# Prisma-pResearch/Deep_Interpolation_Clustering

Measured on AMD Instinct MI355X. Metric: encounters/sec per joint interp+DEC step, higher is better.
Workload: dtype bf16; 1 GPU; 75000 synthetic encounters/GPU, 6 vitals, ~50 irregular samples per channel per 24h (T=96), R=24, K=4, loss ae_mse+10*kl [BASELINE.json configs[1]]; every epoch walks the WHOLE cohort behind a fresh permutation: 3 batches of 32768 incl. the last of 9464 (no drop_last, as upstream); value = encounters stepped / s; ms_per_step = mean over those steps; per_gpu_batch=32768, global_batch=32768, batches_per_epoch=3, encounters_stepped=16242232, parallelism=single, index_order=shuffled, input=ragged encounter store read in place (208 MB resident)

## Files before the change

deep_interpolation_clustering_amd/csrc/dic_lstmgrad.hip:

```cpp
#include "dic_common.h"

namespace dic {

constexpr int GH = 128;
constexpr int G4 = 4 * GH;
constexpr int XW = 32;
constexpr int TR = 32;
constexpr int NBUF = 3;
#ifndef DIC_DW_DGPAD
#define DIC_DW_DGPAD 64
#endif
constexpr int DG_PITCH = 2 * G4 + DIC_DW_DGPAD;
constexpr int H_PITCH = 2 * GH;
constexpr int X_PITCH = 2 * XW;
constexpr int LDS_DG = TR * DG_PITCH, LDS_H = TR * H_PITCH, LDS_X = TR * X_PITCH;
constexpr int SLOT = LDS_DG + LDS_H + LDS_X;
constexpr int WT_COLS = 19, WT_PITCH = 2 * G4 + 16;
constexpr int LDS_WT = WT_COLS * WT_PITCH;
constexpr int LDS_RED = 2 * 4 * 1024;
constexpr int DW_LDS = NBUF * SLOT + LDS_WT + LDS_RED;

typedef __bf16 bf16x8 __attribute__((ext_vector_type(8)));
typedef short s16x4 __attribute__((ext_vector_type(4)));
typedef short s16x8 __attribute__((ext_vector_type(8)));
typedef float f32x16 __attribute__((ext_vector_type(16)));
typedef float f32x4 __attribute__((ext_vector_type(4)));

struct LstmParams {
    const float* w_ih[2]; const float* w_hh[2]; const float* b_ih[2]; const float* b_hh[2];
};
struct LstmGrads {
    float* w_ih[2]; float* w_hh[2]; float* b_ih[2]; float* b_hh[2];
};

template <typename T>
__global__ __launch_bounds__(256) void lstm_pack_kernel(LstmParams p, int I, int Ip, int bias_col, T* wih, T* whh, T* whh_t, T* bias, T* wih_t) {
    const int n_ih = 2 * G4 * Ip, n_hh = 2 * G4 * GH;
    const int total = n_ih + 2 * n_hh + 2 * G4 + (wih_t ? n_ih : 0);
    for (int i = blockIdx.x * 256 + threadIdx.x; i < total; i += gridDim.x * 256) {
        if (i >= n_ih + 2 * n_hh + 2 * G4) {
            const int j = i - (n_ih + 2 * n_hh + 2 * G4), c = j / (2 * G4), row = j - c * (2 * G4), d = row / G4, g = row - d * G4;
            float v = 0.f;
            if (c < I) v = p.w_ih[d][(size_t)g * I + c];
            else if (c == I && bias_col) v = p.b_ih[d][g] + p.b_hh[d][g];
            wih_t[j] = (T)v;
            continue;
        }
        if (i < n_ih) {
            const int row = i / Ip, c = i - row * Ip, d = row / G4, g = row - d * G4;
            float v = 0.f;
            if (c < I) v = p.w_ih[d][(size_t)g * I + c];
            else if (c == I && bias_col) v = p.b_ih[d][g] + p.b_hh[d][g];
            wih[i] = (T)v;
        } else if (i < n_ih + n_hh) {
            const int j = i - n_ih, d = j / (G4 * GH), k = j - d * (G4 * GH);
            whh[j] = (T)p.w_hh[d][k];
        } else if (i < n_ih + 2 * n_hh) {
            const int j = i - n_ih - n_hh, d = j / (G4 * GH), k = j - d * (G4 * GH), u = k / G4, n = k - u * G4;
            if (whh_t) whh_t[j] = (T)p.w_hh[d][(size_t)n * GH + u];
        } else {
            const int j = i - n_ih - 2 * n_hh, d = j / G4, g = j - d * G4;
            if (bias) bias[j] = (T)(p.b_ih[d][g] + p.b_hh[d][g]);
        }
    }
}

struct DwArgs {
    const __bf16* dg;
    const __bf16* hext;
    const __bf16* x;
    float* partials;
    const __bf16* wih;
    __bf16* dxp;
    int R, B;
};
typedef float f32x4_t __attribute__((ext_vector_type(4)));

__device__ __forceinline__ s16x4 lds_tr16(const unsigned char* p) {
    return __builtin_amdgcn_ds_read_tr16_b64_v4i16((__attribute__((address_space(3))) s16x4*)(p));
}
__device__ __forceinline__ void dma16(const void* sbase, unsigned voff, unsigned lds_dst) {
    unsigned keep;
    asm volatile("s_mov_b32 %0, m0\n\ts_mov_b32 m0, %3\n\ts_nop 0\n\tglobal_load_lds_dwordx4 %1, %2\n\ts_mov_b32 m0, %0"
                 : "=&s"(keep) : "v"(voff), "s"(sbase), "s"(lds_dst) : "memory");
}
__device__ __forceinline__ void dma4(const void* sbase, unsigned voff, unsigned lds_dst) {
    unsigned keep;
    asm volatile("s_mov_b32 %0, m0\n\ts_mov_b32 m0, %3\n\ts_nop 0\n\tglobal_load_lds_dword %1, %2\n\ts_mov_b32 m0, %0"
                 : "=&s"(keep) : "v"(voff), "s"(sbase), "s"(lds_dst) : "memory");
}

template <int XWT>
__global__ __launch_bounds__(512) void lstm_dw_kernel(DwArgs a) {
    static_assert(XWT == 32 || XWT == 64, "packed input rows are 32 or 64 wide");
    constexpr int NBX = XWT / 32, NBN = 4 + NBX;
    constexpr int NWT = GH + XWT;
    constexpr int XP = 2 * XWT, L_X = TR * XP;
    constexpr int SLOTT = LDS_DG + LDS_H + L_X;
    extern __shared__ __align__(16) unsigned char dwsm[];
    const int tid = threadIdx.x, lane = tid & 63;
    const int w = __builtin_amdgcn_readfirstlane(tid >> 6);
    const int dir = blockIdx.y;
    const long nrows = (long)a.R * a.B;
    const int ntiles = (int)((nrows + TR - 1) / TR), nch = gridDim.x;
    const __bf16* hsrc = a.hext + (dir ? (size_t)2 * a.B * 2 * GH + GH : 0);

    f32x16 acc[2][NBN];
#pragma unroll
    for (int mb = 0; mb < 2; ++mb)
#pragma unroll
        for (int nb = 0; nb < NBN; ++nb)
#pragma unroll
            for (int k = 0; k < 16; ++k) acc[mb][nb][k] = 0.f;

    const unsigned lds0 = (unsigned)(size_t)((__attribute__((address_space(3))) unsigned char*)dwsm);
    const unsigned v_dg = lane * 16;
    const unsigned v_h = (lane >> 4) * (2 * GH * 2) + (((lane & 15) ^ ((lane >> 4) << 2)) * 16);
    const unsigned v_x = lane * 4;
    const unsigned v_x64[2] = {(unsigned)((lane >> 5) * 128 + (((lane >> 4) & 1) * 64) + (lane & 15) * 4),
                               (unsigned)((lane >> 5) * 128 + ((((lane >> 4) & 1) ^ 1) * 64) + (lane & 15) * 4)};
    auto request = [&](int tile, int slot) {
        const long r0 = min((long)tile * TR, nrows - TR);
        const unsigned base = lds0 + slot * SLOTT;
#pragma unroll
        for (int p = 0; p < 4; ++p) {
            const int row = p * 8 + w;
            dma16(a.dg + ((size_t)(r0 + row) * 2 + dir) * G4, v_dg, base + row * DG_PITCH);
        }
        dma16(hsrc + (size_t)(r0 + w * 4) * 2 * GH, v_h, base + LDS_DG + w * 4 * H_PITCH);
        if constexpr (XWT == 32) {
            dma4(a.x + (size_t)r0 * XWT + w * 128, v_x, base + LDS_DG + LDS_H + w * 256);
        } else {
#pragma unroll
            for (int i = 0; i < 2; ++i)
                dma4(a.x + (size_t)(r0 + 4 * w + 2 * i) * XWT, v_x64[i], base + LDS_DG + LDS_H + (4 * w + 2 * i) * XP);
        }
    };

    const int kq = (lane & 15) >> 2, kp = lane & 3, cb = (lane >> 4) & 1, hh = lane >> 5;
    const int rowoff = 8 * hh + kq;
    const int pa_off = rowoff * DG_PITCH + (64 * w + 16 * cb + 4 * kp) * 2;
    int px_off[NBX];
#pragma unroll
    for (int nbx = 0; nbx < NBX; ++nbx)
        px_off[nbx] = LDS_DG + LDS_H + rowoff * XP + (XWT == 64 ? ((nbx ^ ((rowoff >> 1) & 1)) * 64) : 0) + (16 * cb + 4 * kp) * 2;
    int ph_off[4];
#pragma unroll
    for (int nb = 0; nb < 4; ++nb) ph_off[nb] = LDS_DG + rowoff * H_PITCH + (((4 * nb + 2 * cb + (kp >> 1)) ^ (kq << 2)) * 16) + (kp & 1) * 8;
    auto frag = [&](const unsigned char* p, int pitch) {
        const s16x4 lo = lds_tr16(p), hi = lds_tr16(p + 4 * pitch);
        s16x8 f;
#pragma unroll
        for (int j = 0; j < 4; ++j) { f[j] = lo[j]; f[4 + j] = hi[j]; }
        return __builtin_bit_cast(bf16x8, f);
    };

    unsigned char* wt = dwsm + NBUF * SLOTT;
    float* red = reinterpret_cast<float*>(wt + LDS_WT);
    const bool want_dx = XWT == 32 && a.wih != nullptr;
    if (want_dx) {
        for (int i = tid; i < WT_COLS * G4; i += 512) {
            const int xc = i / G4, k = i - xc * G4;
            *reinterpret_cast<__bf16*>(wt + xc * WT_PITCH + k * 2) = a.wih[((size_t)dir * G4 + k) * XWT + xc];
        }
    }
    const int q4 = w & 3, rw = q4 >> 1, xcb = q4 & 1, khalf = w >> 2, li = lane & 15, kq4 = lane >> 4;
    const int dxa_off = (16 * rw + li) * DG_PITCH + (khalf * 256 + 8 * kq4) * 2;
    const int dxb_off = min(16 * xcb + li, WT_COLS - 1) * WT_PITCH + (khalf * 256 + 8 * kq4) * 2;
    long prev_r0 = -1;
    int parity = 0;
    f32x4_t own_prev = {0.f, 0.f, 0.f, 0.f};
    auto finish_dx = [&](int par, long r0p) {
        if (want_dx && khalf == 0 && r0p >= 0) {
            const f32x4_t o = *reinterpret_cast<const f32x4_t*>(red + (par * 4 + q4) * 256 + lane * 4);
            __bf16* dst = a.dxp + ((size_t)dir * nrows + r0p + 16 * rw + 4 * kq4) * XWT + 16 * xcb + li;
#pragma unroll
            for (int e = 0; e < 4; ++e) dst[(size_t)e * XWT] = (__bf16)(o[e] + own_prev[e]);
        }
    };

    int tile = blockIdx.x, slot = 0;
    if (tile < ntiles) request(tile, 0);
    if (tile + nch < ntiles) request(tile + nch, 1);
    for (; tile < ntiles; tile += nch) {
        if (tile + nch < ntiles) {
            if constexpr (XWT == 32) asm volatile("s_waitcnt vmcnt(6) lgkmcnt(0)" ::: "memory");
            else asm volatile("s_waitcnt vmcnt(7) lgkmcnt(0)" ::: "memory");
        } else {
            asm volatile("s_waitcnt vmcnt(0) lgkmcnt(0)" ::: "memory");
        }
        __builtin_amdgcn_s_barrier();
        finish_dx(parity ^ 1, prev_r0);
        if (tile + 2 * nch < ntiles) request(tile + 2 * nch, slot == 0 ? 2 : slot - 1);
        unsigned char* base = dwsm + slot * SLOTT;
        if ((long)tile * TR + TR > nrows) {
            const int dup = (int)((long)tile * TR + TR - nrows);
            for (int i = tid; i < dup * (H_PITCH + XP) / 16; i += 512) {
                const int nh = dup * H_PITCH / 16;
                unsigned char* dst = i < nh ? base + LDS_DG + i * 16 : base + LDS_DG + LDS_H + (i - nh) * 16;
                *reinterpret_cast<uint4*>(dst) = make_uint4(0u, 0u, 0u, 0u);
            }
            asm volatile("s_waitcnt lgkmcnt(0)" ::: "memory");
            __builtin_amdgcn_s_barrier();
        }
#pragma unroll 1
        for (int ks = 0; ks < TR / 16; ++ks) {
            const unsigned char* kb = base + ks * 16 * DG_PITCH;
            bf16x8 af[2];
#pragma unroll
            for (int mb = 0; mb < 2; ++mb) af[mb] = frag(kb + pa_off + mb * 64, DG_PITCH);
#pragma unroll
            for (int nb = 0; nb < NBN; ++nb) {
                const bf16x8 bfg = nb < 4 ? frag(base + ks * 16 * H_PITCH + ph_off[nb < 4 ? nb : 0], H_PITCH)
                                          : frag(base + ks * 16 * XP + px_off[nb < 4 ? 0 : nb - 4], XP);
#pragma unroll
                for (int mb = 0; mb < 2; ++mb) acc[mb][nb] = __builtin_amdgcn_mfma_f32_32x32x16_bf16(af[mb], bfg, acc[mb][nb], 0, 0, 0);
            }
        }
        if (want_dx) {
            f32x4_t dacc = {0.f, 0.f, 0.f, 0.f};
#pragma unroll
            for (int ks = 0; ks < 8; ++ks) {
                const bf16x8 av = *reinterpret_cast<const bf16x8*>(base + dxa_off + ks * 64);
                const bf16x8 bv = *reinterpret_cast<const bf16x8*>(wt + dxb_off + ks * 64);
                dacc = __builtin_amdgcn_mfma_f32_16x16x32_bf16(av, bv, dacc, 0, 0, 0);
            }
            if (khalf) *reinterpret_cast<f32x4_t*>(red + (parity * 4 + q4) * 256 + lane * 4) = dacc;
            else own_prev = dacc;
            prev_r0 = min((long)tile * TR, nrows - TR);
            parity ^= 1;
        }
        slot = slot == NBUF - 1 ? 0 : slot + 1;
    }
    if (want_dx) {
        asm volatile("s_waitcnt lgkmcnt(0)" ::: "memory");
        __builtin_amdgcn_s_barrier();
        finish_dx(parity ^ 1, prev_r0);
    }
    float* o = a.partials + ((size_t)blockIdx.x * 2 + dir) * G4 * NWT;
#pragma unroll
    for (int mb = 0; mb < 2; ++mb)
#pragma unroll
        for (int nb = 0; nb < NBN; ++nb)
#pragma unroll
            for (int k = 0; k < 16; ++k) {
                const int m = 64 * w + 32 * mb + (k & 3) + 8 * (k >> 2) + 4 * hh;
                o[(size_t)m * NWT + 32 * nb + (lane & 31)] = acc[mb][nb][k];
            }
}

constexpr int DXW = 256;
constexpr int DNW = GH + DXW;
constexpr int DMH = G4 / 2;
static_assert(DNW / 32 == 12, "12 n-blocks = 2 wave groups x 6");
constexpr int WD_DG = TR * DMH * 2, WD_H = TR * GH * 2, WD_X = TR * DXW * 2;
constexpr int WD_SLOT = WD_DG + WD_H + WD_X;
constexpr int WD_LDS = NBUF * WD_SLOT;
constexpr int WD_OUT = 4 * DMH * DNW;

struct DwWideArgs {
    const __bf16* dg;
    const __bf16* hext;
    const __bf16* x;
    float* partials;
    int R, B;
    int x_relu;
};

__global__ __launch_bounds__(512) void lstm_dw_wide_kernel(DwWideArgs a) {
    extern __shared__ __align__(16) unsigned char dwsm[];
    const int tid = threadIdx.x, lane = tid & 63;
    const int w = __builtin_amdgcn_readfirstlane(tid >> 6);
    const int dir = blockIdx.y >> 1, mh = blockIdx.y & 1;
    const long nrows = (long)a.R * a.B;
    const int ntiles = (int)((nrows + TR - 1) / TR), nch = gridDim.x;
    const __bf16* hsrc = a.hext + (dir ? (size_t)2 * a.B * 2 * GH + GH : 0);
    const __bf16* gsrc = a.dg + (size_t)dir * G4 + mh * DMH;

    const int mg = w & 3, ng = w >> 2;
    f32x16 acc[2][6];
#pragma unroll
    for (int mb = 0; mb < 2; ++mb)
#pragma unroll
        for (int nb = 0; nb < 6; ++nb)
#pragma unroll
            for (int k = 0; k < 16; ++k) acc[mb][nb][k] = 0.f;

    const unsigned lds0 = (unsigned)(size_t)((__attribute__((address_space(3))) unsigned char*)dwsm);
    const int r2 = lane >> 5, sw2 = ((2 * (w & 1) + r2) & 3) << 2;
    const unsigned v_dg = r2 * (2 * G4 * 2) + (((lane & 31) ^ sw2) * 16);
    const unsigned v_x = r2 * (DXW * 2) + (((lane & 31) ^ sw2) * 16);
    const unsigned v_h = (lane >> 4) * (2 * GH * 2) + (((lane & 15) ^ ((lane >> 4) << 2)) * 16);
    auto request = [&](int tile, int slot) {
        const long r0 = min((long)tile * TR, nrows - TR);
        const unsigned base = lds0 + slot * WD_SLOT;
#pragma unroll
        for (int p = 0; p < 2; ++p) {
            const int row = 2 * (w + 8 * p);
            dma16(gsrc + (size_t)(r0 + row) * 2 * G4, v_dg, base + row * (DMH * 2));
            dma16(a.x + (size_t)(r0 + row) * DXW, v_x, base + WD_DG + WD_H + row * (DXW * 2));
        }
        dma16(hsrc + (size_t)(r0 + w * 4) * 2 * GH, v_h, base + WD_DG + w * 4 * (GH * 2));
    };

    const int kq = (lane & 15) >> 2, kp = lane & 3, cb = (lane >> 4) & 1, hh = lane >> 5;
    const int rowoff = 8 * hh + kq;
    auto piece = [&](int j) { return (((4 * j + 2 * cb + (kp >> 1)) ^ (kq << 2)) * 16) + (kp & 1) * 8; };
    int pa_off[2], pb_off[6], pb_pitch[6];
    short pb_floor[6];
#pragma unroll
    for (int mb = 0; mb < 2; ++mb) pa_off[mb] = rowoff * (DMH * 2) + piece(2 * mg + mb);
#pragma unroll
    for (int i = 0; i < 6; ++i) {
        const int j = 6 * ng + i;
        pb_pitch[i] = j < 4 ? GH * 2 : DXW * 2;
        pb_floor[i] = (j >= 4 && a.x_relu) ? (short)0 : (short)-32768;
        pb_off[i] = j < 4 ? WD_DG + rowoff * (GH * 2) + piece(j) : WD_DG + WD_H + rowoff * (DXW * 2) + piece(j - 4);
    }
    auto frag = [&](const unsigned char* p, int pitch) {
        const s16x4 lo = lds_tr16(p), hi = lds_tr16(p + 4 * pitch);
        s16x8 f;
#pragma unroll
        for (int j = 0; j < 4; ++j) { f[j] = lo[j]; f[4 + j] = hi[j]; }
        return __builtin_bit_cast(bf16x8, f);
    };

    int tile = blockIdx.x, slot = 0;
    if (tile < ntiles) request(tile, 0);
    if (tile + nch < ntiles) request(tile + nch, 1);
    for (; tile < ntiles; tile += nch) {
        if (tile + nch < ntiles) asm volatile("s_waitcnt vmcnt(5) lgkmcnt(0)" ::: "memory");
        else asm volatile("s_waitcnt vmcnt(0) lgkmcnt(0)" ::: "memory");
        __builtin_amdgcn_s_barrier();
        if (tile + 2 * nch < ntiles) request(tile + 2 * nch, slot == 0 ? 2 : slot - 1);
        unsigned char* base = dwsm + slot * WD_SLOT;
        if ((long)tile * TR + TR > nrows) {
            const int dup = (int)((long)tile * TR + TR - nrows);
            const int nh = dup * GH * 2 / 16, nx = dup * DXW * 2 / 16;
            for (int i = tid; i < nh + nx; i += 512) {
                unsigned char* dst = i < nh ? base + WD_DG + i * 16 : base + WD_DG + WD_H + (i - nh) * 16;
                *reinterpret_cast<uint4*>(dst) = make_uint4(0u, 0u, 0u, 0u);
            }
            asm volatile("s_waitcnt lgkmcnt(0)" ::: "memory");
            __builtin_amdgcn_s_barrier();
        }
#ifdef DIC_DWW_EXP_NOMMA
        const int nks = a.R < 0 ? 1 : 0;
#else
        const int nks = TR / 16;
#endif
#pragma unroll 1
        for (int ks = 0; ks < nks; ++ks) {
            bf16x8 af[2];
#pragma unroll
            for (int mb = 0; mb < 2; ++mb) af[mb] = frag(base + ks * 16 * (DMH * 2) + pa_off[mb], DMH * 2);
#pragma unroll
            for (int i = 0; i < 6; ++i) {
                bf16x8 bfg = frag(base + ks * 16 * pb_pitch[i] + pb_off[i], pb_pitch[i]);
                {
                    typedef short s16x8v __attribute__((ext_vector_type(8)));
                    const short fl = pb_floor[i];
                    const s16x8v flv = {fl, fl, fl, fl, fl, fl, fl, fl};
                    bfg = __builtin_bit_cast(bf16x8, __builtin_elementwise_max(__builtin_bit_cast(s16x8v, bfg), flv));
                }
#pragma unroll
                for (int mb = 0; mb < 2; ++mb) acc[mb][i] = __builtin_amdgcn_mfma_f32_32x32x16_bf16(af[mb], bfg, acc[mb][i], 0, 0, 0);
            }
        }
        slot = slot == NBUF - 1 ? 0 : slot + 1;
    }
    float* o = a.partials + ((size_t)blockIdx.x * 4 + blockIdx.y) * DMH * DNW;
#pragma unroll
    for (int mb = 0; mb < 2; ++mb)
#pragma unroll
        for (int i = 0; i < 6; ++i)
#pragma unroll
            for (int k = 0; k < 16; ++k) {
                const int m = 64 * mg + 32 * mb + (k & 3) + 8 * (k >> 2) + 4 * hh;
                o[(size_t)m * DNW + 32 * (6 * ng + i) + (lane & 31)] = acc[mb][i][k];
            }
}

__global__ __launch_bounds__(256) void lstm_dw_wide_finalize(const float* partials, int nch, LstmGrads g, float beta) {
    const int i = (blockIdx.x * 256 + threadIdx.x) * 4;
    if (i >= WD_OUT) return;
    double ch[8][4];
#pragma unroll
    for (int k = 0; k < 8; ++k)
#pragma unroll
        for (int e = 0; e < 4; ++e) ch[k][e] = 0.0;
    const float* src = partials + i;
    int b = 0;
    for (; b + 8 <= nch; b += 8) {
        float4 v[8];
#pragma unroll
        for (int k = 0; k < 8; ++k) v[k] = *reinterpret_cast<const float4*>(src + (size_t)(b + k) * WD_OUT);
#pragma unroll
        for (int k = 0; k < 8; ++k) { ch[k][0] += (double)v[k].x; ch[k][1] += (double)v[k].y; ch[k][2] += (double)v[k].z; ch[k][3] += (double)v[k].w; }
    }
    for (; b < nch; ++b) {
        const float4 v = *reinterpret_cast<const float4*>(src + (size_t)b * WD_OUT);
        ch[0][0] += (double)v.x; ch[0][1] += (double)v.y; ch[0][2] += (double)v.z; ch[0][3] += (double)v.w;
    }
    const int part = i / (DMH * DNW), rem = i - part * (DMH * DNW), m = (part & 1) * DMH + rem / DNW, n = rem % DNW, d = part >> 1;
    float* dst = n < GH ? g.w_hh[d] + (size_t)m * GH + n : g.w_ih[d] + (size_t)m * DXW + (n - GH);
#pragma unroll
    for (int e = 0; e < 4; ++e) {
        const double s = ((ch[0][e] + ch[1][e]) + (ch[2][e] + ch[3][e])) + ((ch[4][e] + ch[5][e]) + (ch[6][e] + ch[7][e]));
        dst[e] = beta != 0.f ? fmaf(beta, dst[e], (float)s) : (float)s;
    }
}
static_assert(WD_OUT % 4 == 0 && DNW % 4 == 0 && GH % 4 == 0, "four outputs per thread");

static int dw_wide_chunks(int R, int B) {
    const int ntiles = (int)(((long)R * B + TR - 1) / TR);
    const int n = max(1, min(ntiles, kNumCU / 4));
    return n >= 8 ? n / 8 * 8 : n;
}

__global__ __launch_bounds__(256) void lstm_dw_finalize(const float* partials, int nch, int I, int nw, LstmGrads g, float beta) {
    __shared__ double red[256];
    const int n_out = 2 * G4 * nw;
    const double s = reduce_partials_32x8(partials, nch, n_out, blockIdx.x * 32, red);
    const int i = blockIdx.x * 32 + threadIdx.x;
    if (threadIdx.x >= 32 || i >= n_out) return;
    const int d = i / (G4 * nw), rem = i - d * (G4 * nw), m = rem / nw, n = rem - m * nw;
    float* dst;
    if (n < GH) dst = g.w_hh[d] + (size_t)m * GH + n;
    else if (n - GH < I) dst = g.w_ih[d] + (size_t)m * I + (n - GH);
    else return;
    *dst = beta != 0.f ? fmaf(beta, *dst, (float)s) : (float)s;
}

__global__ __launch_bounds__(256) void lstm_unpack_grads_kernel(const float* dw_ih, int ldw, const float* dw_hh, const float* dbias,
                                                               int I, LstmGrads g, float beta) {
    const int n_ih = dw_ih ? 2 * G4 * I : 0, n_hh = dw_hh ? 2 * G4 * GH : 0, n_b = dbias ? 2 * G4 : 0;
    for (int i = blockIdx.x * 256 + threadIdx.x; i < n_ih + n_hh + n_b; i += gridDim.x * 256) {
        if (i < n_ih) {
            const int row = i / I, c = i - row * I, d = row / G4, m = row - d * G4;
            float* dst = g.w_ih[d] + (size_t)m * I + c;
            const float v = dw_ih[(size_t)row * ldw + c];
            *dst = beta != 0.f ? fmaf(beta, *dst, v) : v;
        } else if (i < n_ih + n_hh) {
            const int j = i - n_ih, d = j / (G4 * GH), k = j - d * (G4 * GH);
            float* dst = g.w_hh[d] + k;
            *dst = beta != 0.f ? fmaf(beta, *dst, dw_hh[j]) : dw_hh[j];
        } else {
            const int j = i - n_ih - n_hh, d = j / G4, m = j - d * G4;
            const float v = dbias[j];
            float* d1 = g.b_ih[d] + m;
            float* d2 = g.b_hh[d] + m;
            *d1 = beta != 0.f ? fmaf(beta, *d1, v) : v;
            *d2 = beta != 0.f ? fmaf(beta, *d2, v) : v;
        }
    }
}

constexpr int TX = 16;
template <int XWT, int DMH> struct DwX3 {
    static constexpr int NG = G4 / DMH;
    static constexpr int MW = DMH / 64;
    static constexpr int NBT = 4 + XWT / 32;
    static constexpr int NBN = (NBT + NG - 1) / NG;
    static constexpr int NWT = GH + XWT;
    static constexpr int DGP = DMH == G4 ? 2 * DMH + 64 : 2 * DMH;
    static constexpr int L_PL = TX * DGP, L_DG = 2 * L_PL;
    static constexpr int HP = 2 * GH + 64;
    static constexpr int XP = XWT == 32 ? 64 : 2 * XWT + 64;
    static constexpr int L_H = TX * HP, L_X = TX * XP;
    static constexpr int L_HX = 2 * L_H + 2 * L_X;
    static constexpr int L_RED = XWT == 32 ? 2 * 8 * 1024 : 0;
    static constexpr int LDS = 3 * L_DG + 2 * L_HX + L_RED;
    static constexpr int NXL = XWT == 32 ? 1 : 2;
    static constexpr int NDMA = DMH == G4 ? 4 : 2;
};

struct DwX3Args {
    const __bf16* dg;
    long dg_plane;
    const float* hext;
    const float* x;
    int ldx;
    float* partials;
    int R, B, x_relu;
    const float* wih;
    float* dxp;
};

__device__ __forceinline__ f32x4_t gload16(const void* sbase, unsigned voff) {
    f32x4_t v;
    asm volatile("global_load_dwordx4 %0, %1, %2" : "=&v"(v) : "v"(voff), "s"(sbase) : "memory");
    return v;
}
__device__ __forceinline__ void split4_store(unsigned char* hi, unsigned char* lo, f32x4_t v, bool relu, bool zero) {
    bf16x8 dummy; (void)dummy;
    typedef __bf16 b4 __attribute__((ext_vector_type(4)));
    b4 h, l;
#pragma unroll
    for (int j = 0; j < 4; ++j) {
        float x = zero ? 0.f : v[j];
        if (relu) x = fmaxf(x, 0.f);
        const __bf16 xh = (__bf16)x;
        h[j] = xh;
        l[j] = (__bf16)(x - (float)xh);
    }
    *reinterpret_cast<b4*>(hi) = h;
    *reinterpret_cast<b4*>(lo) = l;
}

#ifdef DIC_DWX3_EXP_TIMING
__device__ unsigned long long dic_dwx3_stamps[8][32][8];
#define DWX_STAMP(tile, slot)                                                                                         \
    do {                                                                                                              \
        if (blockIdx.x == 5 && blockIdx.y == 0 && (threadIdx.x & 63) == 0 && (tile) >= 8 && (tile) < 40)               \
            dic_dwx3_stamps[threadIdx.x >> 6][(tile) - 8][slot] = __builtin_readcyclecounter();                        \
    } while (0)
#else
#define DWX_STAMP(tile, slot) do {} while (0)
#endif

template <int XWT, int DMH>
__global__ __launch_bounds__(512) void lstm_dwx3_kernel(DwX3Args a) {
    typedef DwX3<XWT, DMH> C;
    extern __shared__ __align__(16) unsigned char dwsm[];
    const int tid = threadIdx.x, lane = tid & 63;
    const int w = __builtin_amdgcn_readfirstlane(tid >> 6);
    const int dir = blockIdx.y / C::NG, mh = blockIdx.y % C::NG;
    const int mg = w % C::MW, ng = w / C::MW;
    const long nrows = (long)a.R * a.B;
    const int ntiles = (int)((nrows + TX - 1) / TX), nch = gridDim.x;
    const int mine = (int)blockIdx.x < ntiles ? (ntiles - 1 - (int)blockIdx.x) / nch + 1 : 0;
    if (mine == 0) return;
    const float* hsrc = a.hext + (dir ? (size_t)2 * a.B * 2 * GH + GH : 0);
    const __bf16* gsrc = a.dg + (size_t)dir * G4 + mh * DMH;

    f32x16 acc[2][C::NBN];
#pragma unroll
    for (int mb = 0; mb < 2; ++mb)
#pragma unroll
        for (int nb = 0; nb < C::NBN; ++nb)
#pragma unroll
            for (int k = 0; k < 16; ++k) acc[mb][nb][k] = 0.f;

    unsigned char* const hx0 = dwsm + 3 * C::L_DG;
    const unsigned lds0 = (unsigned)(size_t)((__attribute__((address_space(3))) unsigned char*)dwsm);
    auto tile_r0 = [&](int j) { return min((long)((int)blockIdx.x + min(j, mine - 1) * nch) * TX, nrows - TX); };
    const int r2 = lane >> 5, sw2 = ((2 * (w & 1) + r2) & 3) << 2;
    const unsigned v_dg = DMH == G4 ? (unsigned)lane * 16 : (unsigned)(r2 * (2 * G4 * 2) + (((lane & 31) ^ sw2) * 16));
    auto request_dg = [&](int j) {
        const long r0 = tile_r0(j);
        const unsigned base = lds0 + (j % 3) * C::L_DG;
#pragma unroll
        for (int p = 0; p < 2; ++p) {
            const __bf16* src = gsrc + (size_t)p * a.dg_plane;
            if constexpr (DMH == G4) {
#pragma unroll
                for (int k = 0; k < 2; ++k) dma16(src + (size_t)(r0 + w + 8 * k) * 2 * G4, v_dg, base + p * C::L_PL + (w + 8 * k) * C::DGP);
            } else {
                dma16(src + (size_t)(r0 + 2 * w) * 2 * G4, v_dg, base + p * C::L_PL + 2 * w * C::DGP);
            }
        }
    };
    const int hrow = tid >> 5, hc4 = tid & 31;
    const unsigned v_h = (unsigned)(hrow * (2 * GH * 4) + hc4 * 16);
    const int xpc = a.ldx >> 2;
    int xrow[C::NXL], xc4[C::NXL];
    unsigned v_x[C::NXL];
    bool xon[C::NXL];
#pragma unroll
    for (int i = 0; i < C::NXL; ++i) {
        const int p = tid + 512 * i;
        xon[i] = p < TX * xpc;
        const int pc = xon[i] ? p : 0;
        xrow[i] = pc / xpc; xc4[i] = pc - xrow[i] * xpc;
        v_x[i] = (unsigned)((xrow[i] * a.ldx + 4 * xc4[i]) * 4);
    }
    const int h_pos = hrow * C::HP + hc4 * 8;
    int x_pos[C::NXL];
#pragma unroll
    for (int i = 0; i < C::NXL; ++i) x_pos[i] = xrow[i] * C::XP + xc4[i] * 8;
    f32x4_t hreg, xreg[C::NXL];
    auto request_hx = [&](int j) {
        const long r0 = tile_r0(j);
        hreg = gload16(hsrc + (size_t)r0 * 2 * GH, v_h);
#pragma unroll
        for (int i = 0; i < C::NXL; ++i) xreg[i] = gload16(a.x + (size_t)r0 * a.ldx, v_x[i]);
    };
    constexpr int NPIECE = 1 + C::NXL;
    static_assert(NPIECE <= C::NBN, "dwx3: one MFMA group per piece");
    auto store_piece = [&](int j, int pc) {
        const long t0 = (long)((int)blockIdx.x + min(j, mine - 1) * nch) * TX;
        const int dup = (int)max(0L, t0 + TX - nrows);
        unsigned char* base = hx0 + (j & 1) * C::L_HX;
        if (C::NBN >= 6 && dup == 0) {
            if (pc == 0) split4_store(base + h_pos, base + C::L_H + h_pos, hreg, false, false);
            else if (xon[pc - 1]) split4_store(base + 2 * C::L_H + x_pos[pc - 1], base + 2 * C::L_H + C::L_X + x_pos[pc - 1], xreg[pc - 1], a.x_relu != 0, false);
        } else if (pc == 0) {
            split4_store(base + h_pos, base + C::L_H + h_pos, hreg, false, h_pos < dup * C::HP);
        } else {
            const int i = pc - 1;
            if (xon[i]) split4_store(base + 2 * C::L_H + x_pos[i], base + 2 * C::L_H + C::L_X + x_pos[i], xreg[i], a.x_relu != 0, x_pos[i] < dup * C::XP);
        }
    };
    auto store_hx = [&](int j) {
#pragma unroll
        for (int pc = 0; pc < NPIECE; ++pc) store_piece(j, pc);
    };

    const int kq = (lane & 15) >> 2, kp = lane & 3, cb = (lane >> 4) & 1, hh = lane >> 5;
    const int rowoff = 8 * hh + kq;
    auto piece = [&](int j) { return (((4 * j + 2 * cb + (kp >> 1)) ^ (kq << 2)) * 16) + (kp & 1) * 8; };
    int pa_off[2], pb_pitch[C::NBN], pb_lo[C::NBN];
    int pb_sel[C::NBN], pb_soff[C::NBN];
    const int pb_h = rowoff * C::HP + (16 * cb + 4 * kp) * 2, pb_x = 2 * C::L_H + rowoff * C::XP + (16 * cb + 4 * kp) * 2;
#pragma unroll
    for (int mb = 0; mb < 2; ++mb)
        pa_off[mb] = DMH == G4 ? rowoff * C::DGP + (64 * mg + 32 * mb + 16 * cb + 4 * kp) * 2 : rowoff * C::DGP + piece(2 * mg + mb);
#pragma unroll
    for (int i = 0; i < C::NBN; ++i) {
        const int jn = min(C::NBN * ng + i, C::NBT - 1);
        pb_pitch[i] = jn < 4 ? C::HP : C::XP;
        pb_lo[i] = jn < 4 ? C::L_H : C::L_X;
        pb_sel[i] = jn < 4;
        pb_soff[i] = 64 * (jn < 4 ? jn : jn - 4);
    }
    auto pb_off = [&](int i) { return (pb_sel[i] ? pb_h : pb_x) + pb_soff[i]; };
    auto frag = [&](const unsigned char* p, int pitch) {
        const s16x4 lo = lds_tr16(p), hi = lds_tr16(p + 4 * pitch);
        s16x8 f;
#pragma unroll
        for (int j = 0; j < 4; ++j) { f[j] = lo[j]; f[4 + j] = hi[j]; }
        return __builtin_bit_cast(bf16x8, f);
    };

    constexpr bool DXOK = XWT == 32 && C::NG == 2;
    const bool want_dx = DXOK && a.wih != nullptr;
    float* red = reinterpret_cast<float*>(dwsm + 3 * C::L_DG + 2 * C::L_HX);
    bf16x8 wdh[2], wdl[2];
    const int li = lane & 15, kg4 = lane >> 4;
    if (want_dx) {
#pragma unroll
        for (int ks = 0; ks < 2; ++ks)
#pragma unroll
            for (int jj = 0; jj < 8; ++jj) {
                const int col = 16 * ng + li, k = mh * DMH + 64 * mg + 32 * ks + 8 * kg4 + jj;
                const float v = col < a.ldx ? a.wih[((size_t)dir * G4 + k) * a.ldx + col] : 0.f;
                const __bf16 vh = (__bf16)v;
                wdh[ks][jj] = vh;
                wdl[ks][jj] = (__bf16)(v - (float)vh);
            }
    }
    int dxa_off[2];
#pragma unroll
    for (int ks = 0; ks < 2; ++ks) dxa_off[ks] = li * C::DGP + (((8 * mg + 4 * ks + kg4) ^ ((li & 3) << 2)) * 16);
    auto finish_dx = [&](int jprev) {
        if (!want_dx || jprev < 0) return;
        const int row = tid >> 5, col = tid & 31;
        const float* src = red + (jprev & 1) * (8 * 256) + (col >> 4) * (4 * 256) + ((col & 15) + 16 * (row >> 2)) * 4 + (row & 3);
        const float sum = (src[0] + src[256]) + (src[512] + src[768]);
        if (col < a.ldx) a.dxp[((size_t)blockIdx.y * nrows + tile_r0(jprev) + row) * a.ldx + col] = sum;
    };

    if constexpr (XWT == 32) {
        for (int i = tid; i < 2 * C::L_HX / 16; i += 512) reinterpret_cast<uint4*>(hx0)[i] = make_uint4(0u, 0u, 0u, 0u);
        __syncthreads();
    }
    request_hx(0);
    request_dg(0);
    asm volatile("s_waitcnt vmcnt(%0)" :: "i"(C::NDMA) : "memory");
    asm volatile("" : "+v"(hreg));
#pragma unroll
    for (int i = 0; i < C::NXL; ++i) asm volatile("" : "+v"(xreg[i]));
    store_hx(0);
    request_hx(1);
    request_dg(1);
    for (int j = 0; j < mine; ++j) {
        DWX_STAMP(j, 0);
        asm volatile("s_waitcnt vmcnt(%0) lgkmcnt(0)" :: "i"(C::NDMA) : "memory");
        DWX_STAMP(j, 1);
        asm volatile("" : "+v"(hreg));
#pragma unroll
        for (int i = 0; i < C::NXL; ++i) asm volatile("" : "+v"(xreg[i]));
        __builtin_amdgcn_s_barrier();
        DWX_STAMP(j, 2);
        if constexpr (DXOK) finish_dx(j - 1);
        constexpr bool SPREAD = C::NBN >= 6;
        if constexpr (!SPREAD) {
            store_hx(j + 1);
            request_hx(j + 2);
            request_dg(j + 2);
        }
        DWX_STAMP(j, 3);
        DWX_STAMP(j, 4);
        const unsigned char* dgb = dwsm + (j % 3) * C::L_DG;
        const unsigned char* hxb = hx0 + (j & 1) * C::L_HX;
        bf16x8 ah[2], al[2];
#pragma unroll
        for (int mb = 0; mb < 2; ++mb) {
            ah[mb] = frag(dgb + pa_off[mb], C::DGP);
            al[mb] = frag(dgb + C::L_PL + pa_off[mb], C::DGP);
        }
        if constexpr (!SPREAD) {
#pragma unroll
            for (int i = 0; i < C::NBN; ++i) {
                const bf16x8 bh = frag(hxb + pb_off(i), pb_pitch[i]);
                const bf16x8 bl = frag(hxb + pb_off(i) + pb_lo[i], pb_pitch[i]);
#pragma unroll
                for (int mb = 0; mb < 2; ++mb) {
                    acc[mb][i] = __builtin_amdgcn_mfma_f32_32x32x16_bf16(ah[mb], bh, acc[mb][i], 0, 0, 0);
                    acc[mb][i] = __builtin_amdgcn_mfma_f32_32x32x16_bf16(al[mb], bh, acc[mb][i], 0, 0, 0);
                    acc[mb][i] = __builtin_amdgcn_mfma_f32_32x32x16_bf16(ah[mb], bl, acc[mb][i], 0, 0, 0);
                }
            }
        } else {
            bf16x8 bh = frag(hxb + pb_off(0), pb_pitch[0]);
            bf16x8 bl = frag(hxb + pb_off(0) + pb_lo[0], pb_pitch[0]);
    #pragma unroll
            for (int i = 0; i < C::NBN; ++i) {
                __builtin_amdgcn_sched_barrier(0);
    #pragma unroll
                for (int mb = 0; mb < 2; ++mb) acc[mb][i] = __builtin_amdgcn_mfma_f32_32x32x16_bf16(ah[mb], bh, acc[mb][i], 0, 0, 0);
    #pragma unroll
                for (int mb = 0; mb < 2; ++mb) acc[mb][i] = __builtin_amdgcn_mfma_f32_32x32x16_bf16(al[mb], bh, acc[mb][i], 0, 0, 0);
                __builtin_amdgcn_sched_barrier(0);
                if (i + 1 < C::NBN) bh = frag(hxb + pb_off(i + 1), pb_pitch[i + 1]);
                if constexpr (SPREAD) {
                    if (i < NPIECE) store_piece(j + 1, i);
                    if (i == NPIECE - 1) {
                        request_hx(j + 2);
                        request_dg(j + 2);
                    }
                }
                __builtin_amdgcn_sched_barrier(0);
    #pragma unroll
                for (int mb = 0; mb < 2; ++mb) acc[mb][i] = __builtin_amdgcn_mfma_f32_32x32x16_bf16(ah[mb], bl, acc[mb][i], 0, 0, 0);
                __builtin_amdgcn_sched_barrier(0);
                if (i + 1 < C::NBN) bl = frag(hxb + pb_off(i + 1) + pb_lo[i + 1], pb_pitch[i + 1]);
            }
            __builtin_amdgcn_sched_barrier(0);
        }
        DWX_STAMP(j, 5);
        if constexpr (DXOK) {
            if (want_dx) {
                f32x4_t d0 = {0.f, 0.f, 0.f, 0.f};
#pragma unroll
                for (int ks = 0; ks < 2; ++ks) {
                    const bf16x8 avh = *reinterpret_cast<const bf16x8*>(dgb + dxa_off[ks]);
                    const bf16x8 avl = *reinterpret_cast<const bf16x8*>(dgb + C::L_PL + dxa_off[ks]);
                    d0 = __builtin_amdgcn_mfma_f32_16x16x32_bf16(avh, wdh[ks], d0, 0, 0, 0);
                    d0 = __builtin_amdgcn_mfma_f32_16x16x32_bf16(avl, wdh[ks], d0, 0, 0, 0);
                    d0 = __builtin_amdgcn_mfma_f32_16x16x32_bf16(avh, wdl[ks], d0, 0, 0, 0);
                }
                *reinterpret_cast<f32x4_t*>(red + (j & 1) * (8 * 256) + (ng * 4 + mg) * 256 + lane * 4) = d0;
            }
        }
    }
    asm volatile("s_waitcnt vmcnt(0)" ::: "memory");
    if constexpr (DXOK) {
        if (want_dx) {
            asm volatile("s_waitcnt lgkmcnt(0)" ::: "memory");
            __builtin_amdgcn_s_barrier();
            finish_dx(mine - 1);
        }
    }
    float* o = a.partials + ((size_t)blockIdx.x * gridDim.y + blockIdx.y) * DMH * C::NWT;
#pragma unroll
    for (int mb = 0; mb < 2; ++mb)
#pragma unroll
        for (int i = 0; i < C::NBN; ++i) {
            if (C::NBN * ng + i >= C::NBT) continue;
#pragma unroll
            for (int k = 0; k < 16; ++k) {
                const int m = 64 * mg + 32 * mb + (k & 3) + 8 * (k >> 2) + 4 * hh;
                o[(size_t)m * C::NWT + 32 * (C::NBN * ng + i) + (lane & 31)] = acc[mb][i][k];
            }
        }
}

static int dw_chunks(int R, int B) {
    const int ntiles = (int)(((long)R * B + TR - 1) / TR);
    return max(1, min(ntiles, kNumCU / 2));
}
static int dwx3_chunks(int R, int B, bool wide) {
    const int ntiles = (int)(((long)R * B + TX - 1) / TX);
    (void)wide;
    const int n = max(1, min(ntiles, kNumCU / 4));
    return n >= 8 ? n / 8 * 8 : n;
}

}

using namespace dic;

extern "C" {

int dic_lstm_pack(int dtype, const float* const* params, int H, int I, int Ip, int bias_col, void* wih, void* whh, void* whh_t, void* bias,
                  void* wih_t, dic_stream_t stream) {
    DIC_REQUIRE(dtype == DIC_DTYPE_F32 || dtype == DIC_DTYPE_BF16, DIC_ERR_INVALID_ARG, "lstm_pack: dtype %d", dtype);
    DIC_REQUIRE(H == GH, DIC_ERR_UNSUPPORTED, "lstm_pack: hidden size %d (compiled for %d)", H, GH);
    DIC_REQUIRE(params && wih && whh, DIC_ERR_INVALID_ARG, "lstm_pack: NULL pointer");
    DIC_REQUIRE(I > 0 && Ip >= I + (bias_col ? 1 : 0) && Ip <= 1024, DIC_ERR_INVALID_ARG, "lstm_pack: I=%d Ip=%d bias_col=%d", I, Ip, bias_col);
    LstmParams p;
    for (int d = 0; d < 2; ++d) {
        p.w_ih[d] = params[4 * d + 0]; p.w_hh[d] = params[4 * d + 1]; p.b_ih[d] = params[4 * d + 2]; p.b_hh[d] = params[4 * d + 3];
        DIC_REQUIRE(p.w_ih[d] && p.w_hh[d] && p.b_ih[d] && p.b_hh[d], DIC_ERR_INVALID_ARG, "lstm_pack: NULL parameter (direction %d)", d);
    }
    const int total = 2 * G4 * Ip + 4 * G4 * GH + 2 * G4 + (wih_t ? 2 * G4 * Ip : 0);
    const dim3 grid(min((total + 255) / 256, 2 * kNumCU));
    if (dtype == DIC_DTYPE_BF16)
        hipLaunchKernelGGL(lstm_pack_kernel<__bf16>, grid, dim3(256), 0, (hipStream_t)stream, p, I, Ip, bias_col, (__bf16*)wih, (__bf16*)whh,
                           (__bf16*)whh_t, (__bf16*)bias, (__bf16*)wih_t);
    else
        hipLaunchKernelGGL(lstm_pack_kernel<float>, grid, dim3(256), 0, (hipStream_t)stream, p, I, Ip, bias_col, (float*)wih, (float*)whh,
                           (float*)whh_t, (float*)bias, (float*)wih_t);
    return check_launch("lstm_pack");
}

static int grads_from(float* const* grads, LstmGrads* g, bool need_w, bool need_b, const char* who) {
    DIC_REQUIRE(grads, DIC_ERR_INVALID_ARG, "%s: grads is NULL", who);
    for (int d = 0; d < 2; ++d) {
        g->w_ih[d] = grads[4 * d + 0]; g->w_hh[d] = grads[4 * d + 1]; g->b_ih[d] = grads[4 * d + 2]; g->b_hh[d] = grads[4 * d + 3];
        DIC_REQUIRE(!need_w || (g->w_ih[d] && g->w_hh[d]), DIC_ERR_INVALID_ARG, "%s: NULL weight gradient (direction %d)", who, d);
        DIC_REQUIRE(!need_b || (g->b_ih[d] && g->b_hh[d]), DIC_ERR_INVALID_ARG, "%s: NULL bias gradient (direction %d)", who, d);
    }
    return DIC_OK;
}

size_t dic_lstm_dw_workspace(int R, int B) {
    if (R <= 0 || B <= 0) return 0;
    return (size_t)dw_chunks(R, B) * 2 * G4 * (GH + 64) * sizeof(float);
}

int dic_lstm_dw(const void* dgx, const void* out_ext, const void* x, const void* wih, void* dx_parts, int R, int B, int H, int I, int Ip,
                float* const* grads, int accumulate, void* workspace, size_t workspace_bytes, dic_stream_t stream) {
    DIC_REQUIRE(R > 0 && B > 0, DIC_ERR_INVALID_ARG, "lstm_dw: non-positive size");
    DIC_REQUIRE(H == GH, DIC_ERR_UNSUPPORTED, "lstm_dw: hidden size %d (compiled for %d)", H, GH);
    DIC_REQUIRE((Ip == XW || Ip == 64) && I > 0 && I <= Ip, DIC_ERR_UNSUPPORTED, "lstm_dw: packed input width %d / %d (compiled for %d and 64)", I, Ip, XW);
    DIC_REQUIRE(dgx && out_ext && x && workspace, DIC_ERR_INVALID_ARG, "lstm_dw: NULL pointer");
    DIC_REQUIRE((long)R * B >= TR, DIC_ERR_UNSUPPORTED, "lstm_dw: R*B = %ld rows < one %d-row tile (use the GEMM path)", (long)R * B, TR);
    LstmGrads g;
    int rc = grads_from(grads, &g, true, false, "lstm_dw");
    if (rc) return rc;
    const int nch = dw_chunks(R, B);
    const int wide = Ip == 64, nw = GH + Ip, n_out = 2 * G4 * nw;
    DIC_REQUIRE(workspace_bytes >= (size_t)nch * n_out * sizeof(float), DIC_ERR_WORKSPACE, "lstm_dw: workspace %zu < %zu", workspace_bytes,
                (size_t)nch * n_out * sizeof(float));
    const int lds = wide ? NBUF * (LDS_DG + LDS_H + TR * 2 * 64) : DW_LDS;
    static bool attr_set[2] = {false, false};
    if (!attr_set[wide]) {
        hipError_t e = hipFuncSetAttribute(wide ? (const void*)lstm_dw_kernel<64> : (const void*)lstm_dw_kernel<32>, hipFuncAttributeMaxDynamicSharedMemorySize, lds);
        DIC_REQUIRE(e == hipSuccess, DIC_ERR_LAUNCH, "lstm_dw: cannot reserve %d B of LDS: %s", lds, hipGetErrorString(e));
        attr_set[wide] = true;
    }
    hipStream_t st = (hipStream_t)stream;
    DIC_REQUIRE((wih == nullptr) == (dx_parts == nullptr), DIC_ERR_INVALID_ARG, "lstm_dw: wih and dx_parts go together");
    DIC_REQUIRE(!wih || (!wide && I <= WT_COLS), DIC_ERR_UNSUPPORTED, "lstm_dw: the fused input gradient covers %d input columns of 32-wide rows, got %d of %d", WT_COLS, I, Ip);
    DwArgs a{(const __bf16*)dgx, (const __bf16*)out_ext, (const __bf16*)x, (float*)workspace, (const __bf16*)wih, (__bf16*)dx_parts, R, B};
    if (wide) hipLaunchKernelGGL(lstm_dw_kernel<64>, dim3(nch, 2), dim3(512), lds, st, a);
    else hipLaunchKernelGGL(lstm_dw_kernel<32>, dim3(nch, 2), dim3(512), lds, st, a);
    hipLaunchKernelGGL(lstm_dw_finalize, dim3((n_out + 31) / 32), dim3(256), 0, st, (const float*)workspace, nch, I, nw, g,
                       accumulate ? 1.0f : 0.0f);
    return check_launch("lstm_dw");
}

size_t dic_lstm_dw_wide_workspace(int R, int B) {
    if (R <= 0 || B <= 0) return 0;
    return (size_t)dw_wide_chunks(R, B) * WD_OUT * sizeof(float);
}

int dic_lstm_dw_wide(const void* dgx, const void* out_ext, const void* x, int x_relu, int R, int B, int H, int I, float* const* grads, int accumulate,
                     void* workspace, size_t workspace_bytes, dic_stream_t stream) {
    DIC_REQUIRE(R > 0 && B > 0, DIC_ERR_INVALID_ARG, "lstm_dw_wide: non-positive size");
    DIC_REQUIRE(H == GH, DIC_ERR_UNSUPPORTED, "lstm_dw_wide: hidden size %d (compiled for %d)", H, GH);
    DIC_REQUIRE(I == DXW, DIC_ERR_UNSUPPORTED, "lstm_dw_wide: input width %d (compiled for %d)", I, DXW);
    DIC_REQUIRE(dgx && out_ext && x && workspace, DIC_ERR_INVALID_ARG, "lstm_dw_wide: NULL pointer");
    DIC_REQUIRE((long)R * B >= TR, DIC_ERR_UNSUPPORTED, "lstm_dw_wide: R*B = %ld rows < one %d-row tile (use the GEMM path)", (long)R * B, TR);
    LstmGrads g;
    int rc = grads_from(grads, &g, true, false, "lstm_dw_wide");
    if (rc) return rc;
    const int nch = dw_wide_chunks(R, B);
    DIC_REQUIRE(workspace_bytes >= (size_t)nch * WD_OUT * sizeof(float), DIC_ERR_WORKSPACE, "lstm_dw_wide: workspace %zu < %zu", workspace_bytes,
                (size_t)nch * WD_OUT * sizeof(float));
    static bool attr_set = false;
    if (!attr_set) {
        hipError_t e = hipFuncSetAttribute((const void*)lstm_dw_wide_kernel, hipFuncAttributeMaxDynamicSharedMemorySize, WD_LDS);
        DIC_REQUIRE(e == hipSuccess, DIC_ERR_LAUNCH, "lstm_dw_wide: cannot reserve %d B of LDS: %s", WD_LDS, hipGetErrorString(e));
        attr_set = true;
    }
    hipStream_t st = (hipStream_t)stream;
    DwWideArgs a{(const __bf16*)dgx, (const __bf16*)out_ext, (const __bf16*)x, (float*)workspace, R, B, x_relu != 0};
    hipLaunchKernelGGL(lstm_dw_wide_kernel, dim3(nch, 4), dim3(512), WD_LDS, st, a);
    hipLaunchKernelGGL(lstm_dw_wide_finalize, dim3((WD_OUT / 4 + 255) / 256), dim3(256), 0, st, (const float*)workspace, nch, g, accumulate ? 1.0f : 0.0f);
    return check_launch("lstm_dw_wide");
}

size_t dic_lstm_dw_x3_workspace(int R, int B, int I) {
    if (R <= 0 || B <= 0 || I <= 0) return 0;
    const bool wide = I == DXW;
    return (size_t)dwx3_chunks(R, B, wide) * (wide ? (size_t)WD_OUT : (size_t)2 * G4 * (GH + XW)) * sizeof(float);
}

int dic_lstm_dw_x3(const void* dg_hi, long dg_plane, const float* out_ext, const float* x, int ldx, int x_relu, const float* wih, float* dx_parts, int R, int B, int H,
                   int I, float* const* grads, int accumulate, void* workspace, size_t workspace_bytes, dic_stream_t stream) {
    DIC_REQUIRE(R > 0 && B > 0, DIC_ERR_INVALID_ARG, "lstm_dw_x3: non-positive size");
    DIC_REQUIRE(H == GH, DIC_ERR_UNSUPPORTED, "lstm_dw_x3: hidden size %d (compiled for %d)", H, GH);
    const bool wide = I == DXW;
    DIC_REQUIRE(wide ? ldx == DXW : (I > 0 && I <= ldx && ldx <= XW && ldx % 4 == 0), DIC_ERR_UNSUPPORTED,
                "lstm_dw_x3: input width %d in rows of %d (compiled for %d, or up to %d in rows that are a multiple of 4)", I, ldx, DXW, XW);
    DIC_REQUIRE(dg_hi && dg_plane > 0 && out_ext && x && workspace, DIC_ERR_INVALID_ARG, "lstm_dw_x3: NULL pointer / plane stride");
    DIC_REQUIRE(((uintptr_t)dg_hi & 15) == 0 && dg_plane % 8 == 0 && ((uintptr_t)out_ext & 15) == 0 && ((uintptr_t)x & 15) == 0, DIC_ERR_UNSUPPORTED,
                "lstm_dw_x3: operands must be 16-B aligned");
    DIC_REQUIRE((long)R * B >= TX, DIC_ERR_UNSUPPORTED, "lstm_dw_x3: R*B = %ld rows < one %d-row tile (use the GEMM path)", (long)R * B, TX);
    DIC_REQUIRE((wih == nullptr) == (dx_parts == nullptr) && (!wih || !wide), DIC_ERR_INVALID_ARG, "lstm_dw_x3: wih and dx_parts go together (narrow input only)");
    LstmGrads g;
    int rc = grads_from(grads, &g, true, false, "lstm_dw_x3");
    if (rc) return rc;
    const int nch = dwx3_chunks(R, B, wide);
    DIC_REQUIRE(workspace_bytes >= dic_lstm_dw_x3_workspace(R, B, I), DIC_ERR_WORKSPACE, "lstm_dw_x3: workspace %zu < %zu", workspace_bytes,
                dic_lstm_dw_x3_workspace(R, B, I));
    hipStream_t st = (hipStream_t)stream;
    DwX3Args a{(const __bf16*)dg_hi, dg_plane, out_ext, x, ldx, (float*)workspace, R, B, x_relu != 0, wih, dx_parts};
    static bool attr_set[2] = {false, false};
    const int lds = wide ? DwX3<DXW, G4 / 2>::LDS : DwX3<XW, G4 / 2>::LDS;
    if (!attr_set[wide]) {
        hipError_t e = hipFuncSetAttribute(wide ? (const void*)lstm_dwx3_kernel<DXW, G4 / 2> : (const void*)lstm_dwx3_kernel<XW, G4 / 2>,
                                           hipFuncAttributeMaxDynamicSharedMemorySize, lds);
        DIC_REQUIRE(e == hipSuccess, DIC_ERR_LAUNCH, "lstm_dw_x3: cannot reserve %d B of LDS: %s", lds, hipGetErrorString(e));
        attr_set[wide] = true;
    }
    if (wide) {
        hipLaunchKernelGGL((lstm_dwx3_kernel<DXW, G4 / 2>), dim3(nch, 4), dim3(512), lds, st, a);
        hipLaunchKernelGGL(lstm_dw_wide_finalize, dim3((WD_OUT / 4 + 255) / 256), dim3(256), 0, st, (const float*)workspace, nch, g, accumulate ? 1.0f : 0.0f);
    } else {
        const int nw = GH + XW, n_out = 2 * G4 * nw;
        hipLaunchKernelGGL((lstm_dwx3_kernel<XW, G4 / 2>), dim3(nch, 4), dim3(512), lds, st, a);
        hipLaunchKernelGGL(lstm_dw_finalize, dim3((n_out + 31) / 32), dim3(256), 0, st, (const float*)workspace, nch, I, nw, g, accumulate ? 1.0f : 0.0f);
    }
    return check_launch("lstm_dw_x3");
}

int dic_lstm_unpack_grads(const float* dw_ih, int ldw, const float* dw_hh, const float* dbias, int H, int I, float* const* grads,
                          int accumulate, dic_stream_t stream) {
    DIC_REQUIRE(H == GH, DIC_ERR_UNSUPPORTED, "lstm_unpack_grads: hidden size %d (compiled for %d)", H, GH);
    DIC_REQUIRE(I > 0 && (!dw_ih || ldw >= I), DIC_ERR_INVALID_ARG, "lstm_unpack_grads: I=%d ldw=%d", I, ldw);
    LstmGrads g;
    int rc = grads_from(grads, &g, dw_ih || dw_hh, dbias != nullptr, "lstm_unpack_grads");
    if (rc) return rc;
    const int total = (dw_ih ? 2 * G4 * I : 0) + (dw_hh ? 2 * G4 * GH : 0) + (dbias ? 2 * G4 : 0);
    if (total == 0) return DIC_OK;
    hipLaunchKernelGGL(lstm_unpack_grads_kernel, dim3(min((total + 255) / 256, 2 * kNumCU)), dim3(256), 0, (hipStream_t)stream, dw_ih, ldw,
                       dw_hh, dbias, I, g, accumulate ? 1.0f : 0.0f);
    return check_launch("lstm_unpack_grads");
}

#ifdef DIC_DWX3_EXP_TIMING
int dic_dwx3_debug_stamps(unsigned long long* host) {
    return (int)hipMemcpyFromSymbol(host, HIP_SYMBOL(dic_dwx3_stamps), sizeof(unsigned long long) * 8 * 32 * 8);
}
#endif

}
```

Measured before the change: 5.580 million encounters/s.

## Software-pipeline LDS fragment loads against MFMAs in wide LSTM weight-grad kernel

Result: no change. 5.631 million encounters/s (median of 6 runs) (+0.9%).

```diff
diff --git a/deep_interpolation_clustering_amd/csrc/dic_lstmgrad.hip b/deep_interpolation_clustering_amd/csrc/dic_lstmgrad.hip
--- a/deep_interpolation_clustering_amd/csrc/dic_lstmgrad.hip
+++ b/deep_interpolation_clustering_amd/csrc/dic_lstmgrad.hip
@@ -267,17 +267,16 @@
     int x_relu;
 };
 
-__global__ __launch_bounds__(512) void lstm_dw_wide_kernel(DwWideArgs a) {
-    extern __shared__ __align__(16) unsigned char dwsm[];
+template <int NG>
+__device__ __forceinline__ void dw_wide_body(const DwWideArgs& a, unsigned char* dwsm, const int w) {
     const int tid = threadIdx.x, lane = tid & 63;
-    const int w = __builtin_amdgcn_readfirstlane(tid >> 6);
     const int dir = blockIdx.y >> 1, mh = blockIdx.y & 1;
     const long nrows = (long)a.R * a.B;
     const int ntiles = (int)((nrows + TR - 1) / TR), nch = gridDim.x;
     const __bf16* hsrc = a.hext + (dir ? (size_t)2 * a.B * 2 * GH + GH : 0);
     const __bf16* gsrc = a.dg + (size_t)dir * G4 + mh * DMH;
 
-    const int mg = w & 3, ng = w >> 2;
+    const int mg = w & 3;
     f32x16 acc[2][6];
 #pragma unroll
     for (int mb = 0; mb < 2; ++mb)
@@ -306,17 +305,17 @@
     const int kq = (lane & 15) >> 2, kp = lane & 3, cb = (lane >> 4) & 1, hh = lane >> 5;
     const int rowoff = 8 * hh + kq;
     auto piece = [&](int j) { return (((4 * j + 2 * cb + (kp >> 1)) ^ (kq << 2)) * 16) + (kp & 1) * 8; };
-    int pa_off[2], pb_off[6], pb_pitch[6];
-    short pb_floor[6];
+    int pa_off[2], pb_off[6];
 #pragma unroll
     for (int mb = 0; mb < 2; ++mb) pa_off[mb] = rowoff * (DMH * 2) + piece(2 * mg + mb);
 #pragma unroll
     for (int i = 0; i < 6; ++i) {
-        const int j = 6 * ng + i;
-        pb_pitch[i] = j < 4 ? GH * 2 : DXW * 2;
-        pb_floor[i] = (j >= 4 && a.x_relu) ? (short)0 : (short)-32768;
+        const int j = 6 * NG + i;
         pb_off[i] = j < 4 ? WD_DG + rowoff * (GH * 2) + piece(j) : WD_DG + WD_H + rowoff * (DXW * 2) + piece(j - 4);
     }
+    typedef short s16x8v __attribute__((ext_vector_type(8)));
+    const short xfl = a.x_relu ? (short)0 : (short)-32768;
+    const s16x8v xfloor = {xfl, xfl, xfl, xfl, xfl, xfl, xfl, xfl};
     auto frag = [&](const unsigned char* p, int pitch) {
         const s16x4 lo = lds_tr16(p), hi = lds_tr16(p + 4 * pitch);
         s16x8 f;
@@ -332,7 +331,7 @@
         if (tile + nch < ntiles) asm volatile("s_waitcnt vmcnt(5) lgkmcnt(0)" ::: "memory");
         else asm volatile("s_waitcnt vmcnt(0) lgkmcnt(0)" ::: "memory");
         __builtin_amdgcn_s_barrier();
-        if (tile + 2 * nch < ntiles) request(tile + 2 * nch, slot == 0 ? 2 : slot - 1);
+        const bool more = tile + 2 * nch < ntiles;
         unsigned char* base = dwsm + slot * WD_SLOT;
         if ((long)tile * TR + TR > nrows) {
             const int dup = (int)((long)tile * TR + TR - nrows);
@@ -345,27 +344,38 @@
             __builtin_amdgcn_s_barrier();
         }
 #ifdef DIC_DWW_EXP_NOMMA
-        const int nks = a.R < 0 ? 1 : 0;
-#else
-        const int nks = TR / 16;
+        if (a.R >= 0) {
+            if (more) request(tile + 2 * nch, slot == 0 ? 2 : slot - 1);
+            slot = slot == NBUF - 1 ? 0 : slot + 1;
+            continue;
+        }
 #endif
-#pragma unroll 1
-        for (int ks = 0; ks < nks; ++ks) {
-            bf16x8 af[2];
-#pragma unroll
-            for (int mb = 0; mb < 2; ++mb) af[mb] = frag(base + ks * 16 * (DMH * 2) + pa_off[mb], DMH * 2);
-#pragma unroll
-            for (int i = 0; i < 6; ++i) {
-                bf16x8 bfg = frag(base + ks * 16 * pb_pitch[i] + pb_off[i], pb_pitch[i]);
-                {
-                    typedef short s16x8v __attribute__((ext_vector_type(8)));
-                    const short fl = pb_floor[i];
-                    const s16x8v flv = {fl, fl, fl, fl, fl, fl, fl, fl};
-                    bfg = __builtin_bit_cast(bf16x8, __builtin_elementwise_max(__builtin_bit_cast(s16x8v, bfg), flv));
-                }
-#pragma unroll
-                for (int mb = 0; mb < 2; ++mb) acc[mb][i] = __builtin_amdgcn_mfma_f32_32x32x16_bf16(af[mb], bfg, acc[mb][i], 0, 0, 0);
-            }
+        constexpr int NP = 2 * 6, DIST = 3;
+        auto lda = [&](int ks, int mb) { return frag(base + ks * 16 * (DMH * 2) + pa_off[mb], DMH * 2); };
+        auto ldb = [&](int p) {
+            const int ks = p / 6, i = p % 6, pitch = 6 * NG + i < 4 ? GH * 2 : DXW * 2;
+            return frag(base + ks * 16 * pitch + pb_off[i], pitch);
+        };
+        bf16x8 af[2][2], bq[DIST + 1];
+        af[0][0] = lda(0, 0);
+        af[0][1] = lda(0, 1);
+#pragma unroll
+        for (int p = 0; p < DIST; ++p) bq[p] = ldb(p);
+        __builtin_amdgcn_sched_barrier(0);
+        if (more) request(tile + 2 * nch, slot == 0 ? 2 : slot - 1);
+        __builtin_amdgcn_sched_barrier(0);
+#pragma unroll
+        for (int p = 0; p < NP; ++p) {
+            const int ks = p / 6, i = p % 6;
+            if (p + DIST < NP) bq[(p + DIST) % (DIST + 1)] = ldb(p + DIST);
+            if (p == 1 || p == 2) af[1][p - 1] = lda(1, p - 1);
+            __builtin_amdgcn_sched_barrier(0);
+            bf16x8 bfg = bq[p % (DIST + 1)];
+            if (6 * NG + i >= 4)
+                bfg = __builtin_bit_cast(bf16x8, __builtin_elementwise_max(__builtin_bit_cast(s16x8v, bfg), xfloor));
+#pragma unroll
+            for (int mb = 0; mb < 2; ++mb) acc[mb][i] = __builtin_amdgcn_mfma_f32_32x32x16_bf16(af[ks][mb], bfg, acc[mb][i], 0, 0, 0);
+            __builtin_amdgcn_sched_barrier(0);
         }
         slot = slot == NBUF - 1 ? 0 : slot + 1;
     }
@@ -377,8 +387,15 @@
 #pragma unroll
             for (int k = 0; k < 16; ++k) {
                 const int m = 64 * mg + 32 * mb + (k & 3) + 8 * (k >> 2) + 4 * hh;
-                o[(size_t)m * DNW + 32 * (6 * ng + i) + (lane & 31)] = acc[mb][i][k];
-            }
+                o[(size_t)m * DNW + 32 * (6 * NG + i) + (lane & 31)] = acc[mb][i][k];
+            }
+}
+
+__global__ __launch_bounds__(512) void lstm_dw_wide_kernel(DwWideArgs a) {
+    extern __shared__ __align__(16) unsigned char dwsm[];
+    const int w = __builtin_amdgcn_readfirstlane(threadIdx.x >> 6);
+    if (w < 4) dw_wide_body<0>(a, dwsm, w);
+    else dw_wide_body<1>(a, dwsm, w);
 }
 
 __global__ __launch_bounds__(256) void lstm_dw_wide_finalize(const float* partials, int nch, LstmGrads g, float beta) {
```
